# Gorilla-Lab-SCUT/DCL-Net

Measured on AMD Instinct MI355X. Metric: frames/sec DCL_Net.forward @ YCB-V bs32, higher is better.
Workload: dtype f32 (exact 3xbf16-split products on the bf16 MFMA, f32 accumulate)

## Files before the change

### dcl-net_amd/csrc/linear_split.hip

```cpp
#include <hip/hip_runtime.h>
#include "common.h"
#include "linear_epilogue.h"

namespace {

constexpr int kSpKC = 16;
constexpr int kSpBM = 256, kSpBN = 128;
constexpr int kSpA = kSpBM * kSpKC * 4;
constexpr int kSpP = kSpBN * kSpKC * 2;
constexpr int kSpB = 3 * kSpP;
constexpr int kSpST = kSpA + kSpB;

struct LinSplitArgs {
  const float *x;
  const unsigned char *planes;
  const float *bias;
  float *y;
  long long ldx, ldy;
  int M, N, K, relu;
  const float *roww;
  int rows_per_crop;
  long long w_stride;
  float *part;
  const float *b3;
  long long ldp;
  int xcd_remap;
};

__global__ __launch_bounds__(256) void k_split_weight(const float *__restrict__ Wt, long long ldw, int K, int N, unsigned *__restrict__ planes) {
  const int ntn = (N + kSpBN - 1) / kSpBN;
  const long long pieces = (long long)(K / kSpKC) * ntn * kSpBN * 2;
  for (long long i = blockIdx.x * 256ll + threadIdx.x; i < pieces; i += (long long)gridDim.x * 256) {
    const int hs = (int)(i & 1), c = (int)((i >> 1) & (kSpBN - 1));
    const long long ct = i >> 8;
    const int kc = (int)(ct / ntn), tn = (int)(ct - (long long)kc * ntn);
    const int hh = hs ^ ((c >> 3) & 1), col = tn * kSpBN + c, k0 = kc * kSpKC + 8 * hh;
    unsigned h[4], m[4], l[4];
#pragma unroll
    for (int e = 0; e < 4; ++e) {
      const float w0 = col < N ? Wt[(size_t)(k0 + 2 * e) * ldw + col] : 0.0f, w1 = col < N ? Wt[(size_t)(k0 + 2 * e + 1) * ldw + col] : 0.0f;
      bf16_split2(w0, w1, h[e], m[e], l[e]);
    }
    unsigned *dst = planes + (size_t)ct * (kSpB / 4) + (size_t)(c * 2 + hs) * 4;
#pragma unroll
    for (int e = 0; e < 4; ++e) { dst[e] = h[e]; dst[kSpP / 4 + e] = m[e]; dst[2 * (kSpP / 4) + e] = l[e]; }
  }
}

template <int EPI>
__global__ __launch_bounds__(256, 2) void k_linear_split(const LinSplitArgs a) {
  extern __shared__ __attribute__((aligned(16))) unsigned char sp_lds[];
  const int ntn = (a.N + kSpBN - 1) / kSpBN, ntm = (a.M + kSpBM - 1) / kSpBM, tiles = ntm * ntn;
  int t_lo, t_hi, t_stride;
  xcd_tile_range(a.xcd_remap & 1, tiles, t_lo, t_hi, t_stride);
  const int tid = threadIdx.x, lane = tid & 63, wave = __builtin_amdgcn_readfirstlane(tid >> 6);
  const int r = lane & 31, h = lane >> 5;
  const int nchunks = a.K / kSpKC;
  const int whatif = a.xcd_remap >> 1;
  const unsigned lds0 = lds_addr(sp_lds);
  const size_t bstep = (size_t)ntn * kSpB;

  const int asw = (r >> 2) & 3;
  const unsigned char *afrag = sp_lds + (wave * 64 + r) * 64;
  const unsigned char *bfrag = sp_lds + kSpA + r * 32 + ((h ^ ((r >> 3) & 1)) << 4);

  for (int tile = t_lo; tile < t_hi; tile += t_stride) {
    const int tm = tile / ntn, tn = tile - tm * ntn;
    const int row0 = tm * kSpBM, col0 = tn * kSpBN;
    unsigned aoff[4];
#pragma unroll
    for (int i = 0; i < 4; ++i) {
      const int row = wave * 64 + i * 16 + (lane >> 2);
      const int p = (lane & 3) ^ ((row >> 2) & 3);
      const int srow = min(row0 + row, a.M - 1) - row0;
      aoff[i] = (unsigned)(((long long)srow * a.ldx + 4 * p) * 4);
    }
    const unsigned boff = (unsigned)tid * 16u;
    const float *abase = a.x + (size_t)row0 * a.ldx;
    const unsigned char *bbase = a.planes + (size_t)tn * kSpB;
    auto issue_piece = [&](int k, int stage) {
      const unsigned s0 = lds0 + (unsigned)(stage * kSpST);
      if (k < 3) glds16_s(boff + (unsigned)(k * 4096), bbase, s0 + (unsigned)(kSpA + k * 4096 + wave * 1024));
      else glds16_s(aoff[k - 3], abase, s0 + (unsigned)((wave * 64 + (k - 3) * 16) * 64));
      if (k == 6) { abase += kSpKC; bbase += bstep; }
    };
    auto issue = [&](int stage) {
#pragma unroll
      for (int k = 0; k < 7; ++k) issue_piece(k, stage);
    };
    f32x16 acc[2][4];
#pragma unroll
    for (int i = 0; i < 2; ++i)
#pragma unroll
      for (int j = 0; j < 4; ++j)
#pragma unroll
        for (int e = 0; e < 16; ++e) acc[i][j][e] = 0.0f;

    dcl_lds_barrier();
    if constexpr (EPI == 1) {
      float *wl = reinterpret_cast<float *>(sp_lds + 2 * kSpST);
      const int row = row0 + tid, crop = row / a.rows_per_crop;
      wl[tid] = row < a.M ? a.roww[(size_t)crop * a.w_stride + (row - crop * a.rows_per_crop)] : 0.0f;
    }
    issue(0);
    asm volatile("s_waitcnt vmcnt(0)" ::: "memory");
    for (int c = 0; c < nchunks; ++c) {
      const int st = c & 1;
      asm volatile("s_waitcnt lgkmcnt(0)" ::: "memory");
      __builtin_amdgcn_s_barrier();
      const bool more = c + 1 < nchunks;
      const unsigned char *sa = afrag + st * kSpST, *sb = bfrag + st * kSpST;
      float4 av[2][2];
      u32x4 ap[2][3], bp[4][3];
      auto read_a = [&](int i) {
#pragma unroll
        for (int q = 0; q < 2; ++q) av[i][q] = *reinterpret_cast<const float4 *>(sa + i * 32 * 64 + (((2 * h + q) ^ asw) << 4));
      };
      auto read_b = [&](int j) {
#pragma unroll
        for (int p = 0; p < 3; ++p) bp[j][p] = *reinterpret_cast<const u32x4 *>(sb + p * kSpP + j * 32 * 32);
      };
      auto split_a = [&](int i, int part) {
        unsigned ph, pm, pl;
        const float4 v = av[i][part >> 1];
        if (part & 1) bf16_split2(v.z, v.w, ph, pm, pl); else bf16_split2(v.x, v.y, ph, pm, pl);
        ap[i][0][part] = ph; ap[i][1][part] = pm; ap[i][2][part] = pl;
      };
      read_a(0);
      read_b(0);
      read_a(1);
      if (more && !(whatif & 1)) issue(st ^ 1);
      __builtin_amdgcn_sched_barrier(0);
      if (!(whatif & 2)) {
#pragma unroll
        for (int part = 0; part < 4; ++part) split_a(0, part);
      } else {
#pragma unroll
        for (int p = 0; p < 3; ++p) ap[0][p] = u32x4{__float_as_uint(av[0][0].x), __float_as_uint(av[0][0].y), __float_as_uint(av[0][1].x), __float_as_uint(av[0][1].y)};
      }
      read_b(1);
      __builtin_amdgcn_sched_barrier(0);
#pragma unroll
      for (int blk = 0; blk < 8; ++blk) {
        const int i = blk >> 2, j = blk & 3;
        acc[i][j] = __builtin_amdgcn_mfma_f32_32x32x16_bf16(as_bf16x8(ap[i][2]), as_bf16x8(bp[j][0]), acc[i][j], 0, 0, 0);
        acc[i][j] = __builtin_amdgcn_mfma_f32_32x32x16_bf16(as_bf16x8(ap[i][0]), as_bf16x8(bp[j][2]), acc[i][j], 0, 0, 0);
        acc[i][j] = __builtin_amdgcn_mfma_f32_32x32x16_bf16(as_bf16x8(ap[i][1]), as_bf16x8(bp[j][1]), acc[i][j], 0, 0, 0);
        acc[i][j] = __builtin_amdgcn_mfma_f32_32x32x16_bf16(as_bf16x8(ap[i][1]), as_bf16x8(bp[j][0]), acc[i][j], 0, 0, 0);
        acc[i][j] = __builtin_amdgcn_mfma_f32_32x32x16_bf16(as_bf16x8(ap[i][0]), as_bf16x8(bp[j][1]), acc[i][j], 0, 0, 0);
        acc[i][j] = __builtin_amdgcn_mfma_f32_32x32x16_bf16(as_bf16x8(ap[i][0]), as_bf16x8(bp[j][0]), acc[i][j], 0, 0, 0);
        if (blk < 4) {
          if (!(whatif & 2)) split_a(1, blk);
          else { ap[1][0][blk] = __float_as_uint(av[1][blk >> 1].x); ap[1][1][blk] = __float_as_uint(av[1][blk >> 1].y); ap[1][2][blk] = __float_as_uint(av[1][blk >> 1].z); }
        }
        if (blk < 2) read_b(blk + 2);
        __builtin_amdgcn_sched_barrier(0);
      }
      asm volatile("s_waitcnt vmcnt(0)" ::: "memory");
    }
    asm volatile("s_nop 15\n\ts_nop 7" ::: "memory");

    if constexpr (EPI == 0) {
      if (whatif & 4) continue;
      const bool whole = row0 + kSpBM <= a.M && col0 + kSpBN <= a.N;
      lin_epi_store<true>(acc, a, whole, row0 + wave * 64, col0, r, h);
    } else if constexpr (EPI == 3) {
      unsigned char *vp = reinterpret_cast<unsigned char *>(a.part);
      const int crop = row0 / a.rows_per_crop, key0 = row0 - crop * a.rows_per_crop;
#pragma unroll
      for (int j = 0; j < 4; ++j) {
        const int c = col0 + j * 32 + r;
        const float bias = (a.bias && c < a.N) ? a.bias[c] : 0.0f;
        const int hs = h ^ ((c >> 3) & 1);
#pragma unroll
        for (int i = 0; i < 2; ++i)
#pragma unroll
          for (int hf = 0; hf < 2; ++hf) {
            const long long ht = (long long)crop * a.ldp + ((key0 + wave * 64 + i * 32) >> 4) + hf;
            u32x4 ph, pm, pl;
#pragma unroll
            for (int e = 0; e < 4; ++e) {
              float v0 = acc[i][j][8 * hf + 2 * e] + bias, v1 = acc[i][j][8 * hf + 2 * e + 1] + bias;
              if (a.relu) { v0 = fmaxf(v0, 0.0f); v1 = fmaxf(v1, 0.0f); }
              unsigned qh, qm, ql;
              bf16_split2(v0, v1, qh, qm, ql);
              ph[e] = qh; pm[e] = qm; pl[e] = ql;
            }
            unsigned char *dst = vp + (size_t)ht * (3 * 320 * 32) + (size_t)(c * 2 + hs) * 16;
            if (c < a.N) {
              *reinterpret_cast<u32x4 *>(dst) = ph;
              *reinterpret_cast<u32x4 *>(dst + 320 * 32) = pm;
              *reinterpret_cast<u32x4 *>(dst + 2 * 320 * 32) = pl;
            }
          }
      }
    } else if constexpr (EPI == 2) {
      const float b3 = a.b3[0];
      float *out = a.part;
      const int M = a.M;
      lin_epi_rowdot(acc, a, row0 + wave * 64, col0, r, h, [=](int orow, float sdot) {
        if (r == 0 && orow < M) out[orow] = sdot + b3;
      });
    } else {
      const float *wts = reinterpret_cast<const float *>(sp_lds + 2 * kSpST);
      float *red = reinterpret_cast<float *>(sp_lds + 2 * kSpST) + kSpBM;
      lin_epi_colsum(acc, a, wts, red + wave * kSpBN, wave * 64, col0, 0, r, h);
      dcl_lds_barrier();
      {
        const int pt = tid >> 7, cl = tid & 127;
        if (col0 + cl < a.N && row0 + pt * 128 < a.M)
          a.part[(size_t)(2 * tm + pt) * a.ldp + col0 + cl] = red[(2 * pt) * kSpBN + cl] + red[(2 * pt + 1) * kSpBN + cl];
      }
    }
  }
}

DCL_HOOK_INT(g_sp_xcd, 1);

template <int EPI>
int launch_linear_split(const LinSplitArgs &a, hipStream_t stream) {
  const long long tiles = (long long)((a.M + kSpBM - 1) / kSpBM) * ((a.N + kSpBN - 1) / kSpBN);
  if (tiles > 0x7fffffffll) {
    dcl_set_error("dcl_linear_split_fwd: too many tiles");
    return DCL_EINVAL;
  }
  constexpr size_t lds = (size_t)2 * kSpST + (EPI == 1 ? (kSpBM + 4 * kSpBN) * sizeof(float) : 0);
  static bool attr_set = false;
  if (!attr_set) {
    (void)hipFuncSetAttribute((const void *)k_linear_split<EPI>, hipFuncAttributeMaxDynamicSharedMemorySize, (int)lds);
    attr_set = true;
  }
  hipLaunchKernelGGL((k_linear_split<EPI>), dim3((unsigned)tiles), dim3(256), lds, stream, a);
  return 0;
}

bool lin_split_ok(const float *x, int64_t ldx, const void *planes, int K) {
  return K >= kSpKC && K % kSpKC == 0 && ldx % 4 == 0 && ((size_t)x & 15) == 0 && ((size_t)planes & 15) == 0;
}

}

#ifdef DCL_DIAG
DCL_API void dcl_debug_linear_split_xcd_remap(int on) { g_sp_xcd = ((int)g_sp_xcd & ~1) | (on & 1); }
DCL_API void dcl_debug_linear_split_whatif(int bits) { g_sp_xcd = ((int)g_sp_xcd & 1) | (bits << 1); }
#endif

DCL_API int64_t dcl_linear_split_weight_bytes(int K, int N) {
  if (K <= 0 || N <= 0 || K % kSpKC) return 0;
  return (int64_t)(K / kSpKC) * ((N + kSpBN - 1) / kSpBN) * kSpB;
}

DCL_API int dcl_linear_split_weight(const float *Wt, int64_t ldw, int K, int N, void *planes, dclStream_t stream) {
  DCL_CHECK_ARG(Wt && planes && K > 0 && N > 0 && K % kSpKC == 0 && ldw >= N && ((size_t)planes & 15) == 0);
  const long long pieces = (long long)(K / kSpKC) * ((N + kSpBN - 1) / kSpBN) * kSpBN * 2;
  const unsigned grid = (unsigned)((pieces + 255) / 256 > 4096 ? 4096 : (pieces + 255) / 256);
  hipLaunchKernelGGL(k_split_weight, dim3(grid), dim3(256), 0, (hipStream_t)stream, Wt, (long long)ldw, K, N, (unsigned *)planes);
  DCL_LAUNCH_CHECK();
  return 0;
}

DCL_API int dcl_linear_split_fwd(const float *x, int64_t ldx, const void *planes, const float *bias, float *y, int64_t ldy, int M, int N,
                                 int K, int relu, dclStream_t stream) {
  DCL_CHECK_ARG(M >= 0 && N > 0 && K > 0 && x && planes && y && ldx >= K && ldy >= N);
  DCL_CHECK_ARG(lin_split_ok(x, ldx, planes, K));
  if (M == 0) return 0;
  LinSplitArgs a{x, (const unsigned char *)planes, bias, y, ldx, ldy, M, N, K, relu, nullptr, 1, 0, nullptr, nullptr, 0, (int)g_sp_xcd};
  int rc = launch_linear_split<0>(a, (hipStream_t)stream);
  if (rc) return rc;
  DCL_LAUNCH_CHECK();
  return 0;
}

DCL_API int dcl_linear_split_pool_fwd(const float *x, int64_t ldx, const void *planes, const float *bias, const float *roww,
                                      int rows_per_crop, int64_t w_stride, float *part, int64_t ldp, int M, int N, int K, int relu,
                                      dclStream_t stream) {
  DCL_CHECK_ARG(M > 0 && N > 0 && K > 0 && x && planes && roww && part && ldx >= K && ldp >= N && rows_per_crop >= 1 && w_stride >= 0);
  DCL_CHECK_ARG(lin_split_ok(x, ldx, planes, K));
  LinSplitArgs a{x, (const unsigned char *)planes, bias, nullptr, ldx, 0, M, N, K, relu, roww, rows_per_crop, w_stride, part, nullptr, ldp,
                 (int)g_sp_xcd};
  int rc = launch_linear_split<1>(a, (hipStream_t)stream);
  if (rc) return rc;
  DCL_LAUNCH_CHECK();
  return 0;
}

DCL_API int dcl_linear_split_vpieces_fwd(const float *x, int64_t ldx, const void *planes, const float *bias, void *vplanes,
                                         int rows_per_crop, int M, int N, int K, int relu, dclStream_t stream) {
  DCL_CHECK_ARG(M > 0 && N > 0 && N <= 320 && N % 32 == 0 && K > 0 && x && planes && vplanes && ldx >= K && rows_per_crop > 0);
  DCL_CHECK_ARG(rows_per_crop % kSpBM == 0 && M % rows_per_crop == 0 && (((size_t)vplanes) & 15) == 0);
  DCL_CHECK_ARG(lin_split_ok(x, ldx, planes, K));
  LinSplitArgs a{x, (const unsigned char *)planes, bias, nullptr, ldx, 0, M, N, K, relu, nullptr, rows_per_crop, 0, (float *)vplanes, nullptr,
                 (long long)(rows_per_crop / 16), (int)g_sp_xcd};
  int rc = launch_linear_split<3>(a, (hipStream_t)stream);
  if (rc) return rc;
  DCL_LAUNCH_CHECK();
  return 0;
}

DCL_API int dcl_linear_split_rowdot_fwd(const float *x, int64_t ldx, const void *planes, const float *bias, const float *w3, int64_t ldw3,
                                        const float *b3, float *out, int M, int N, int K, dclStream_t stream) {
  DCL_CHECK_ARG(M >= 0 && N > 0 && N <= kSpBN && K > 0 && x && planes && w3 && b3 && out && ldx >= K && ldw3 >= 1);
  DCL_CHECK_ARG(lin_split_ok(x, ldx, planes, K));
  if (M == 0) return 0;
  LinSplitArgs a{x, (const unsigned char *)planes, bias, nullptr, ldx, 0, M, N, K, 1, w3, 1, ldw3, out, b3, 0, (int)g_sp_xcd};
  int rc = launch_linear_split<2>(a, (hipStream_t)stream);
  if (rc) return rc;
  DCL_LAUNCH_CHECK();
  return 0;
}
```

Baseline: 2124.

## Software-pipeline A-fragment reads and split into previous chunk's MFMA loop

For non-EPI3 variants, the A fragments for the next K-chunk are read from LDS and split into bf16 planes during the tail of the current chunk's MFMA sequence. The global-to-LDS loads are now spread across the MFMA blocks instead of issued all at once, which shortens the serial head of each iteration. The whatif diagnostic becomes a compile-time zero outside DCL_DIAG, so its branches drop out of the default build. The change also calls hipFuncSetAttribute on every launch instead of once, which adds host overhead, and it relies on a partial vmcnt wait and the LDS stage ordering being correct.

Measured after the change: 2160 (median of 6 runs). +1.7%, better.

```diff
diff --git a/dcl-net_amd/csrc/linear_split.hip b/dcl-net_amd/csrc/linear_split.hip
--- a/dcl-net_amd/csrc/linear_split.hip
+++ b/dcl-net_amd/csrc/linear_split.hip
@@ -56,7 +56,11 @@
   const int tid = threadIdx.x, lane = tid & 63, wave = __builtin_amdgcn_readfirstlane(tid >> 6);
   const int r = lane & 31, h = lane >> 5;
   const int nchunks = a.K / kSpKC;
+#ifdef DCL_DIAG
   const int whatif = a.xcd_remap >> 1;
+#else
+  constexpr int whatif = 0;
+#endif
   const unsigned lds0 = lds_addr(sp_lds);
   const size_t bstep = (size_t)ntn * kSpB;
 
@@ -82,11 +86,8 @@
       const unsigned s0 = lds0 + (unsigned)(stage * kSpST);
       if (k < 3) glds16_s(boff + (unsigned)(k * 4096), bbase, s0 + (unsigned)(kSpA + k * 4096 + wave * 1024));
       else glds16_s(aoff[k - 3], abase, s0 + (unsigned)((wave * 64 + (k - 3) * 16) * 64));
-      if (k == 6) { abase += kSpKC; bbase += bstep; }
-    };
-    auto issue = [&](int stage) {
-#pragma unroll
-      for (int k = 0; k < 7; ++k) issue_piece(k, stage);
+      if (k == 2) bbase += bstep;
+      if (k == 6) abase += kSpKC;
     };
     f32x16 acc[2][4];
 #pragma unroll
@@ -95,6 +96,26 @@
       for (int j = 0; j < 4; ++j)
 #pragma unroll
         for (int e = 0; e < 16; ++e) acc[i][j][e] = 0.0f;
+
+    constexpr bool kShortHead = EPI != 3;
+    float4 av[2][2];
+    u32x4 ap[2][3];
+    auto read_a = [&](int i, int stage) {
+      const unsigned char *sa = afrag + stage * kSpST;
+#pragma unroll
+      for (int q = 0; q < 2; ++q) av[i][q] = *reinterpret_cast<const float4 *>(sa + i * 32 * 64 + (((2 * h + q) ^ asw) << 4));
+    };
+    auto split_a = [&](int i, int part) {
+      if (!(whatif & 2)) {
+        unsigned ph, pm, pl;
+        const float4 v = av[i][part >> 1];
+        if (part & 1) bf16_split2(v.z, v.w, ph, pm, pl); else bf16_split2(v.x, v.y, ph, pm, pl);
+        ap[i][0][part] = ph; ap[i][1][part] = pm; ap[i][2][part] = pl;
+      } else {
+        const float4 v = av[i][part >> 1];
+        ap[i][0][part] = __float_as_uint(v.x); ap[i][1][part] = __float_as_uint(v.y); ap[i][2][part] = __float_as_uint(v.z);
+      }
+    };
 
     dcl_lds_barrier();
     if constexpr (EPI == 1) {
@@ -102,43 +123,42 @@
       const int row = row0 + tid, crop = row / a.rows_per_crop;
       wl[tid] = row < a.M ? a.roww[(size_t)crop * a.w_stride + (row - crop * a.rows_per_crop)] : 0.0f;
     }
-    issue(0);
+#pragma unroll
+    for (int k = 0; k < 7; ++k) issue_piece(k, 0);
     asm volatile("s_waitcnt vmcnt(0)" ::: "memory");
+    if constexpr (kShortHead) {
+      read_a(0, 0);
+      read_a(1, 0);
+#pragma unroll
+      for (int part = 0; part < 4; ++part) split_a(0, part);
+    }
     for (int c = 0; c < nchunks; ++c) {
       const int st = c & 1;
       asm volatile("s_waitcnt lgkmcnt(0)" ::: "memory");
       __builtin_amdgcn_s_barrier();
-      const bool more = c + 1 < nchunks;
-      const unsigned char *sa = afrag + st * kSpST, *sb = bfrag + st * kSpST;
-      float4 av[2][2];
-      u32x4 ap[2][3], bp[4][3];
-      auto read_a = [&](int i) {
-#pragma unroll
-        for (int q = 0; q < 2; ++q) av[i][q] = *reinterpret_cast<const float4 *>(sa + i * 32 * 64 + (((2 * h + q) ^ asw) << 4));
-      };
+      const bool more = c + 1 < nchunks, dma = more && !(whatif & 1);
+      const unsigned char *sb = bfrag + st * kSpST;
+      u32x4 bp[4][3];
       auto read_b = [&](int j) {
 #pragma unroll
         for (int p = 0; p < 3; ++p) bp[j][p] = *reinterpret_cast<const u32x4 *>(sb + p * kSpP + j * 32 * 32);
       };
-      auto split_a = [&](int i, int part) {
-        unsigned ph, pm, pl;
-        const float4 v = av[i][part >> 1];
-        if (part & 1) bf16_split2(v.z, v.w, ph, pm, pl); else bf16_split2(v.x, v.y, ph, pm, pl);
-        ap[i][0][part] = ph; ap[i][1][part] = pm; ap[i][2][part] = pl;
-      };
-      read_a(0);
-      read_b(0);
-      read_a(1);
-      if (more && !(whatif & 1)) issue(st ^ 1);
-      __builtin_amdgcn_sched_barrier(0);
-      if (!(whatif & 2)) {
+      if constexpr (kShortHead) {
+        read_b(0);
+        read_b(1);
+      } else {
+        read_a(0, st);
+        read_b(0);
+        read_a(1, st);
+        if (dma) {
+#pragma unroll
+          for (int k = 0; k < 7; ++k) issue_piece(k, st ^ 1);
+        }
+        __builtin_amdgcn_sched_barrier(0);
 #pragma unroll
         for (int part = 0; part < 4; ++part) split_a(0, part);
-      } else {
-#pragma unroll
-        for (int p = 0; p < 3; ++p) ap[0][p] = u32x4{__float_as_uint(av[0][0].x), __float_as_uint(av[0][0].y), __float_as_uint(av[0][1].x), __float_as_uint(av[0][1].y)};
-      }
-      read_b(1);
+        read_b(1);
+      }
       __builtin_amdgcn_sched_barrier(0);
 #pragma unroll
       for (int blk = 0; blk < 8; ++blk) {
@@ -149,11 +169,22 @@
         acc[i][j] = __builtin_amdgcn_mfma_f32_32x32x16_bf16(as_bf16x8(ap[i][1]), as_bf16x8(bp[j][0]), acc[i][j], 0, 0, 0);
         acc[i][j] = __builtin_amdgcn_mfma_f32_32x32x16_bf16(as_bf16x8(ap[i][0]), as_bf16x8(bp[j][1]), acc[i][j], 0, 0, 0);
         acc[i][j] = __builtin_amdgcn_mfma_f32_32x32x16_bf16(as_bf16x8(ap[i][0]), as_bf16x8(bp[j][0]), acc[i][j], 0, 0, 0);
-        if (blk < 4) {
-          if (!(whatif & 2)) split_a(1, blk);
-          else { ap[1][0][blk] = __float_as_uint(av[1][blk >> 1].x); ap[1][1][blk] = __float_as_uint(av[1][blk >> 1].y); ap[1][2][blk] = __float_as_uint(av[1][blk >> 1].z); }
+        if (blk < 4) split_a(1, blk);
+        if (blk < 2) read_b(blk + 2);
+        if (kShortHead && dma) {
+          if (blk == 0) { issue_piece(3, st ^ 1); issue_piece(4, st ^ 1); }
+          if (blk == 1) { issue_piece(5, st ^ 1); issue_piece(6, st ^ 1); }
+          if (blk >= 2 && blk <= 4) issue_piece(blk - 2, st ^ 1);
         }
-        if (blk < 2) read_b(blk + 2);
+        if (kShortHead && more) {
+          if (blk == 5) {
+            asm volatile("s_waitcnt vmcnt(3)" ::: "memory");
+            read_a(0, st ^ 1);
+            read_a(1, st ^ 1);
+          }
+          if (blk == 6) { split_a(0, 0); split_a(0, 1); }
+          if (blk == 7) { split_a(0, 2); split_a(0, 3); }
+        }
         __builtin_amdgcn_sched_barrier(0);
       }
       asm volatile("s_waitcnt vmcnt(0)" ::: "memory");
@@ -225,11 +256,7 @@
     return DCL_EINVAL;
   }
   constexpr size_t lds = (size_t)2 * kSpST + (EPI == 1 ? (kSpBM + 4 * kSpBN) * sizeof(float) : 0);
-  static bool attr_set = false;
-  if (!attr_set) {
-    (void)hipFuncSetAttribute((const void *)k_linear_split<EPI>, hipFuncAttributeMaxDynamicSharedMemorySize, (int)lds);
-    attr_set = true;
-  }
+  (void)hipFuncSetAttribute((const void *)k_linear_split<EPI>, hipFuncAttributeMaxDynamicSharedMemorySize, (int)lds);
   hipLaunchKernelGGL((k_linear_split<EPI>), dim3((unsigned)tiles), dim3(256), lds, stream, a);
   return 0;
 }
```
